# Huiweizhou/GCGCN

Measured on NVIDIA B200. Metric: document graphs/sec (fwd+bwd graph blocks), higher is better.
Workload: dtype f32

## Files before the change

### gcgcn_b200/csrc/gcn_block.cu

```cuda
#include "common.cuh"
#include "mma_tf32.cuh"

namespace gcgcn {

constexpr int BK_THREADS = 256;
constexpr int BK_WARPS = BK_THREADS / WARP;

enum { BK_OUT_DA = 0, BK_OUT_DS = 1, BK_OUT_DQ = 2 };

__device__ __forceinline__ void cp_async16(float* smem_dst, const float* gsrc) {
    const uint32_t d = static_cast<uint32_t>(__cvta_generic_to_shared(smem_dst));
    asm volatile("cp.async.cg.shared.global [%0], [%1], 16;" ::"r"(d), "l"(gsrc) : "memory");
}
__device__ __forceinline__ void cp_async_commit() { asm volatile("cp.async.commit_group;" ::: "memory"); }
template <int N>
__device__ __forceinline__ void cp_async_wait() {
    asm volatile("cp.async.wait_group %0;" ::"n"(N) : "memory");
}

__device__ __forceinline__ uint32_t s_addr(const void* p) { return static_cast<uint32_t>(__cvta_generic_to_shared(p)); }
__device__ __forceinline__ void ldsm4(uint32_t (&r)[4], const float* p) {
    asm volatile("ldmatrix.sync.aligned.m8n8.x4.shared.b16 {%0,%1,%2,%3}, [%4];"
                 : "=r"(r[0]), "=r"(r[1]), "=r"(r[2]), "=r"(r[3])
                 : "r"(s_addr(p))
// ... 194 lines not shown
        for (int r = 0; r < 8; ++r) {
            const int j = L.l8 + 8 * r;
            v[r] = -INFINITY;
            if (r < NT8 && rv && j < n) {
                v[r] = DH > 0 ? Alo[i * LDA + j] : A[abase + static_cast<long long>(i) * n + j];
                m = fmaxf(m, v[r]);
            }
        }
        float inv = 1.f;
        if (DH > 0) {
            m = group8_max(m);
            float z = 0.f;
#pragma unroll
            for (int r = 0; r < 8; ++r) {
                v[r] = (v[r] == -INFINITY) ? 0.f : __expf(v[r] - m);
                z += v[r];
            }
            z = group8_sum(z);
            inv = rv ? 1.0f / z : 0.f;
        }
        float sum = 0.f;
#pragma unroll
        for (int r = 0; r < 8; ++r) {
            const int j = L.l8 + 8 * r;
            if (r < NT8) {
                float p = 0.f;
                if (rv && j < n) {
                    p = v[r] * inv;
                    const long long pidx = abase + static_cast<long long>(i) * n + j;
                    if (DH > 0) P[pidx] = p;
                    if (drop.thr_att != 0u) p *= drop_keep(drop.seed, drop.s_att, pidx, drop.thr_att, drop.inv_att);
                }
                float hi, lo;
                split_f(p, hi, lo);
                Ahi[i * LDA + j] = hi;
                Alo[i * LDA + j] = lo;
                sum += p;
            }
        }
        sum = group8_sum(sum);
        if (L.l8 == 0) rs[i] = 1.0f / (sum + (sum == 0.f ? 1.f : 0.f));
    }

#pragma unroll
    for (int l = 0; l < layers; ++l) {
        float* Zs = Zs0 + (l & 1) * NP * LDZ;
        const int kin = l * GD;
        cp_async_wait<1>();
        __syncthreads();
        const int mt = L.warp / NG, ng = L.warp - mt * NG;
        const bool busy = L.warp < UNITS;
        const int col0 = 8 * NTW * ng;
        float c[NTW][4];
        float* zc = Zs + (16 * mt + L.g) * LDZ + col0 + 2 * L.t;
        if (l > 0) {
            if (busy) {
                const float* wb = Wf + (static_cast<size_t>(h) * layers + l) * (KI * GD * 2) + (col0 / 8) * 128 + L.lane;
#pragma unroll
                for (int nt = 0; nt < NTW; ++nt) {
                    const float2 lo2 = *reinterpret_cast<const float2*>(zc + 8 * nt);
                    const float2 hi2 = *reinterpret_cast<const float2*>(zc + 8 * LDZ + 8 * nt);
                    c[nt][0] = lo2.x; c[nt][1] = lo2.y; c[nt][2] = hi2.x; c[nt][3] = hi2.y;
                }
                const float* pa = Ghi + (16 * mt + L.a_row) * LDG + L.a_col;
#pragma unroll 2
                for (int k0 = 0; k0 < kin; k0 += 8) {
                    uint32_t ah[4], al[4];
                    ldsm4(ah, pa + k0);
                    ldsm4(al, pa + NP * LDG + k0);
#pragma unroll
                    for (int nt = 0; nt < NTW; ++nt) {
                        const float* f = wb + (k0 / 8) * (GD / 8) * 128 + nt * 128;
                        mma3(c[nt], ah, al, __float_as_uint(__ldg(f)), __float_as_uint(__ldg(f + 32)),
                             __float_as_uint(__ldg(f + 64)), __float_as_uint(__ldg(f + 96)));
                    }
                }
#pragma unroll
                for (int nt = 0; nt < NTW; ++nt) {
                    *reinterpret_cast<float2*>(zc + 8 * nt) = make_float2(c[nt][0], c[nt][1]);
                    *reinterpret_cast<float2*>(zc + 8 * LDZ + 8 * nt) = make_float2(c[nt][2], c[nt][3]);
                }
            }
            __syncthreads();
            for (int idx = tid; idx < n * CG; idx += BK_THREADS) {
                const int i = idx / CG, c4 = (idx - i * CG) * 4;
                *reinterpret_cast<float4*>(Z + hbase + (i * HD + kin + c4)) =
                    *reinterpret_cast<const float4*>(Zs + i * LDZ + c4);
            }
        }
        if (busy) {
            float2 e2[2][NTW], x2[2][NTW];
#pragma unroll
            for (int half = 0; half < 2; ++half) {
                const int i = 16 * mt + L.g + 8 * half;
#pragma unroll
                for (int nt = 0; nt < NTW; ++nt) {
                    e2[half][nt] = make_float2(0.f, 0.f);
                    x2[half][nt] = make_float2(0.f, 0.f);
                    if (i < n) {
                        const int col = col0 + 8 * nt + 2 * L.t;
                        e2[half][nt] = ld2g(Eb + (i * HD + kin + col));
                        x2[half][nt] = ld2g(xb + (i * S + kin + col));
                    }
                }
            }
#pragma unroll
            for (int nt = 0; nt < NTW; ++nt) { c[nt][0] = 0.f; c[nt][1] = 0.f; c[nt][2] = 0.f; c[nt][3] = 0.f; }
            const float* pa = Ahi + (16 * mt + L.a_row) * LDA + L.a_col;
            const float* zb = Zs + L.t * LDZ + col0 + L.g;
#pragma unroll
            for (int k0 = 0; k0 < NP; k0 += 8) {
                uint32_t ah[4], al[4];
                ldsm4(ah, pa + k0);
                ldsm4(al, pa + NP * LDA + k0);
#pragma unroll
                for (int nt = 0; nt < NTW; ++nt) mma3f(c[nt], ah, al, zb[k0 * LDZ + 8 * nt], zb[(k0 + 4) * LDZ + 8 * nt]);
            }
#pragma unroll
            for (int half = 0; half < 2; ++half) {
                const int i = 16 * mt + L.g + 8 * half;
                if (i >= n) continue;
                const float rinv = rs[i];
#pragma unroll
                for (int nt = 0; nt < NTW; ++nt) {
                    const int col = col0 + 8 * nt + 2 * L.t;
                    const int off = i * HD + kin + col;
                    float2 o;
                    o.x = fmaxf((e2[half][nt].x + c[nt][2 * half]) * rinv, 0.f);
                    o.y = fmaxf((e2[half][nt].y + c[nt][2 * half + 1]) * rinv, 0.f);
                    *reinterpret_cast<float2*>(Gb + off) = o;
                    float2 f = o;
                    if (drop.thr_gcn != 0u) {
                        const float2 k2 = drop_keep2(drop.seed, drop.s_gcn, hbase + off, drop.thr_gcn, drop.inv_gcn);
                        f.x *= k2.x; f.y *= k2.y;
                    }
                    *reinterpret_cast<float2*>(Fb + off) = make_float2(f.x + x2[half][nt].x, f.y + x2[half][nt].y);
                    if (l < layers - 1) {
                        float2 hi, lo;
                        split_f(o.x, hi.x, lo.x);
                        split_f(o.y, hi.y, lo.y);
                        *reinterpret_cast<float2*>(Ghi + i * LDG + kin + col) = hi;
                        *reinterpret_cast<float2*>(Glo + i * LDG + kin + col) = lo;
                    }
                }
            }
        }
        __syncthreads();
        if (l + 2 < layers) issue_z(l + 2);
        cp_async_commit();
    }
    cp_async_wait<0>();
}

template <int GD, int DH, int OUT, int MTC>
__global__ void __launch_bounds__(BK_THREADS, MTC <= 2 ? 4 : 3)
block_bwd_kernel(const int* __restrict__ node_ptr, const long long* __restrict__ pair_ptr,
                 const float* __restrict__ A, const float* __restrict__ q, const float* __restrict__ Z,
                 const float* __restrict__ G, const float* __restrict__ Wb, const float* __restrict__ dF,
                 float* __restrict__ dZ, float* __restrict__ dE, float* __restrict__ dOut, int heads,
                 long long total_pairs, const int* __restrict__ doc_order, int first, float scale, const BlockDrop drop) {
    extern __shared__ __align__(16) float smem[];
    const int b = doc_order != nullptr ? doc_order[first + blockIdx.x] : blockIdx.x;
    const int h = blockIdx.y;
    const int node0 = node_ptr[b];
    const int n = node_ptr[b + 1] - node0;
    if (n == 0) return;
    constexpr int S = D, layers = D / GD, CG = GD / 4, RPP = BK_THREADS / CG;
    constexpr bool SWZ = (GD == 64);
    constexpr int LDN = SWZ ? GD : GD + 12;
    constexpr int DHH = DH > 0 ? DH : 8;
    constexpr int NTW = col_tiles_per_warp(MTC, GD / 8), NG = (GD / 8) / NTW, UNITS = MTC * NG;
    constexpr int NTW_C = MTC, NG_C = 2, UNITS_C = 2 * MTC;
    constexpr int NP = 16 * MTC, MT = MTC, NT8 = 2 * MTC, LDA = NP + 4, KI = (layers - 1) * GD, LDG = KI + 4;
    const int HD = DH > 0 ? (D / DHH) * S : heads * S;

    constexpr bool TWO = (layers == 2);
    float* AtS = smem;
    float* dNh = AtS + NP * LDA;
    float* dNl = dNh + NP * LDN;
    float* Th = dNl + NP * LDN;
    float* Tl = Th + NP * LDN;
    float* rs = Tl + NP * LDN;
    float* drs = rs + NP;
    float* dAs = TWO ? Tl + NP * LDN - NP * LDA : drs + NP;
    float* dGs = TWO ? dNh : dAs + NP * LDA;
    constexpr int LDP = TWO ? LDN : LDG;

    const int tid = threadIdx.x;
    const LaneGeo L;
    auto pl = [](int row, int col) -> int {
        if (!SWZ) return row * LDN + col;
        const int mask = ((row & 3) << 1) | ((row >> 2) & 1);
        return row * LDN + ((((col >> 2) ^ mask) << 2) | (col & 3));
    };
    const long long abase = static_cast<long long>(h) * total_pairs + pair_ptr[b];
    const float* Ab = A + abase;
    const size_t hbase = static_cast<size_t>(node0) * HD + h * S;

#pragma unroll
    for (int r0 = 0; r0 < NP; r0 += 32) {
        const int i = r0 + L.rsub;
        if (i >= NP) continue;
        float sum = 0.f;
#pragma unroll
        for (int r = 0; r < 8; ++r) {
            const int j = L.l8 + 8 * r;
            if (r < NT8) {
                float v = (i < n && j < n) ? Ab[i * n + j] : 0.f;
                if (drop.thr_att != 0u && i < n && j < n)
                    v *= drop_keep(drop.seed, drop.s_att, abase + i * n + j, drop.thr_att, drop.inv_att);
                AtS[j * LDA + i] = v;
                sum += v;
            }
        }
        sum = group8_sum(sum);
        if (L.l8 == 0) { rs[i] = 1.0f / (sum + (sum == 0.f ? 1.f : 0.f)); drs[i] = 0.f; }
    }
    __syncthreads();

    const int cg = tid % CG, rg = tid / CG, c0 = cg * 4;
    float cA[NTW_C][4];
#pragma unroll
    for (int nt = 0; nt < NTW_C; ++nt) { cA[nt][0] = 0.f; cA[nt][1] = 0.f; cA[nt][2] = 0.f; cA[nt][3] = 0.f; }
#pragma unroll
    for (int l = layers - 1; l >= 0; --l) {
        const float* wsrc = Wb + (static_cast<size_t>(h) * layers + l) * (KI * GD * 2);
        const bool first_layer = (l == layers - 1);
#pragma unroll
        for (int i0 = 0; i0 < NP; i0 += RPP) {
            const int i = i0 + rg;
            if (NP % RPP != 0 && i >= NP) continue;
            float4 dn = make_float4(0.f, 0.f, 0.f, 0.f), zl = dn;
            float drp = 0.f;
            if (i < n) {
                const size_t off = hbase + (i * HD + l * GD + c0);
                float4 dg = ld4g(dF + off);
                const float4 g4 = ld4g(G + off);
                zl = ld4g(Z + off);
                if (drop.thr_gcn != 0u) {
                    const float2 k01 = drop_keep2(drop.seed, drop.s_gcn, off, drop.thr_gcn, drop.inv_gcn);
                    const float2 k23 = drop_keep2(drop.seed, drop.s_gcn, off + 2, drop.thr_gcn, drop.inv_gcn);
                    dg.x *= k01.x; dg.y *= k01.y; dg.z *= k23.x; dg.w *= k23.y;
                }
                if (!first_layer) {
                    const float4 s4 = *reinterpret_cast<const float4*>(dGs + (TWO ? pl(i, l * GD + c0) : i * LDP + l * GD + c0));
                    dg.x += s4.x; dg.y += s4.y; dg.z += s4.z; dg.w += s4.w;
                }
                dg.x = g4.x > 0.f ? dg.x : 0.f; dg.y = g4.y > 0.f ? dg.y : 0.f;
                dg.z = g4.z > 0.f ? dg.z : 0.f; dg.w = g4.w > 0.f ? dg.w : 0.f;
                const float rinv = rs[i];
                dn.x = dg.x * rinv; dn.y = dg.y * rinv; dn.z = dg.z * rinv; dn.w = dg.w * rinv;
                *reinterpret_cast<float4*>(dE + off) = dn;
                drp = -(dn.x * g4.x + dn.y * g4.y + dn.z * g4.z + dn.w * g4.w);
            }
            float4 hi, lo;
            split_f4(dn, hi, lo);
            *reinterpret_cast<float4*>(dNh + pl(i, c0)) = hi;
            *reinterpret_cast<float4*>(dNl + pl(i, c0)) = lo;
            split_f4(zl, hi, lo);
            *reinterpret_cast<float4*>(Th + pl(i, c0)) = hi;
            *reinterpret_cast<float4*>(Tl + pl(i, c0)) = lo;
#pragma unroll
            for (int o = CG / 2; o > 0; o >>= 1) drp += __shfl_xor_sync(0xffffffffu, drp, o);
            if (cg == 0 && i < n) drs[i] += drp;
        }
        __syncthreads();
        if (L.warp < UNITS_C) {
            const int mt = L.warp / NG_C, jg = L.warp - mt * NG_C;
            float (&c)[NTW_C][4] = cA;
            const int arow = 16 * mt + L.a_row, brow = 8 * NTW_C * jg + L.b_row;
            const float* pb = L.b_lo ? Tl : Th;
#pragma unroll
            for (int k0 = 0; k0 < GD; k0 += 8) {
                uint32_t ah[4], al[4];
                const float* pa = dNh + pl(arow, L.a_col + k0);
                ldsm4(ah, pa);
                ldsm4(al, pa + NP * LDN);
                const int boff = pl(brow, L.b_col + k0);
#pragma unroll
                for (int nt = 0; nt < NTW_C; ++nt) {
                    uint32_t bb[4];
                    ldsm4(bb, pb + boff + 8 * nt * LDN);
                    mma3(c[nt], ah, al, bb[0], bb[1], bb[2], bb[3]);
                }
            }
        }
        const int jt = L.warp / NG, ng = L.warp - jt * NG;
        const bool busy = L.warp < UNITS;
        const int col0 = 8 * NTW * ng;
        {
            float c[NTW][4];
#pragma unroll
            for (int nt = 0; nt < NTW; ++nt) { c[nt][0] = 0.f; c[nt][1] = 0.f; c[nt][2] = 0.f; c[nt][3] = 0.f; }
            if (busy) {
                const float* pa = AtS + (16 * jt + L.a_row) * LDA + L.a_col;
#pragma unroll
                for (int k0 = 0; k0 < NP; k0 += 8) {
                    uint32_t ah[4], al[4];
                    ldsm4(ah, pa + k0);
#pragma unroll
                    for (int e = 0; e < 4; ++e) {
                        float hi, lo;
                        split_f(__uint_as_float(ah[e]), hi, lo);
                        ah[e] = __float_as_uint(hi);
                        al[e] = __float_as_uint(lo);
                    }
#pragma unroll
                    for (int nt = 0; nt < NTW; ++nt) {
                        const float* n0 = dNh + pl(k0 + L.t, col0 + 8 * nt + L.g);
                        const float* n1 = dNh + pl(k0 + 4 + L.t, col0 + 8 * nt + L.g);
                        mma3(c[nt], ah, al, __float_as_uint(n0[0]), __float_as_uint(n1[0]), __float_as_uint(n0[NP * LDN]),
                             __float_as_uint(n1[NP * LDN]));
                    }
                }
            }
            __syncthreads();
            if (busy) {
#pragma unroll
                for (int nt = 0; nt < NTW; ++nt)
#pragma unroll
                    for (int half = 0; half < 2; ++half) {
                        const int j = 16 * jt + L.g + 8 * half, col = col0 + 8 * nt + 2 * L.t;
                        const float2 v = make_float2(c[nt][2 * half], c[nt][2 * half + 1]);
                        float2 hi, lo;
                        split_f(v.x, hi.x, lo.x);
                        split_f(v.y, hi.y, lo.y);
                        *reinterpret_cast<float2*>(Th + pl(j, col)) = hi;
                        *reinterpret_cast<float2*>(Tl + pl(j, col)) = lo;
                        if (j < n) *reinterpret_cast<float2*>(dZ + hbase + (j * HD + l * GD + col)) = v;
                    }
            }
        }
        __syncthreads();
        if (busy) {
#pragma unroll
            for (int m = 0; m < l; ++m) {
                float c[NTW][4];
#pragma unroll
                for (int nt = 0; nt < NTW; ++nt) { c[nt][0] = 0.f; c[nt][1] = 0.f; c[nt][2] = 0.f; c[nt][3] = 0.f; }
                const float* wb = wsrc + m * (GD * GD * 2) + (col0 / 8) * 128 + L.lane;
#pragma unroll 2
                for (int k0 = 0; k0 < GD; k0 += 8) {
                    uint32_t ah[4], al[4];
                    const float* pa = Th + pl(16 * jt + L.a_row, L.a_col + k0);
                    ldsm4(ah, pa);
                    ldsm4(al, pa + NP * LDN);
#pragma unroll
                    for (int nt = 0; nt < NTW; ++nt) {
                        const float* f = wb + (k0 / 8) * (GD / 8) * 128 + nt * 128;
                        mma3(c[nt], ah, al, __float_as_uint(__ldg(f)), __float_as_uint(__ldg(f + 32)),
                             __float_as_uint(__ldg(f + 64)), __float_as_uint(__ldg(f + 96)));
                    }
                }
#pragma unroll
                for (int nt = 0; nt < NTW; ++nt)
#pragma unroll
                    for (int half = 0; half < 2; ++half) {
                        float2* p = reinterpret_cast<float2*>(dGs + (TWO ? pl(16 * jt + L.g + 8 * half, m * GD + col0 + 8 * nt + 2 * L.t)
                                                                        : (16 * jt + L.g + 8 * half) * LDP + m * GD + col0 + 8 * nt + 2 * L.t));
                        float2 v = make_float2(c[nt][2 * half], c[nt][2 * half + 1]);
                        if (!first_layer) { const float2 cur = *p; v.x += cur.x; v.y += cur.y; }
                        *p = v;
                    }
            }
        }
        __syncthreads();
    }

    if (L.warp < UNITS_C) {
        const int mt = L.warp / NG_C, jg = L.warp - mt * NG_C;
#pragma unroll
        for (int nt = 0; nt < NTW_C; ++nt)
#pragma unroll
            for (int half = 0; half < 2; ++half)
                *reinterpret_cast<float2*>(dAs + (16 * mt + L.g + 8 * half) * LDA + 8 * (NTW_C * jg + nt) + 2 * L.t) =
                    make_float2(cA[nt][2 * half], cA[nt][2 * half + 1]);
    }
    __syncthreads();
#pragma unroll
    for (int r0 = 0; r0 < NP; r0 += 32) {
        const int i = r0 + L.rsub;
        if (i >= NP) continue;
        const bool rv = i < n;
        const float dr = rv ? drs[i] : 0.f;
        float p[8], dp[8];
        float dot = 0.f;
#pragma unroll
        for (int r = 0; r < 8; ++r) {
            const int j = L.l8 + 8 * r;
            p[r] = 0.f; dp[r] = 0.f;
            if (r < NT8 && rv && j < n) {
                dp[r] = dAs[i * LDA + j] + dr;
                if (OUT != BK_OUT_DA) {
                    if (drop.thr_att != 0u) {
                        dp[r] *= drop_keep(drop.seed, drop.s_att, abase + i * n + j, drop.thr_att, drop.inv_att);
                        p[r] = Ab[i * n + j];
                    } else {
                        p[r] = AtS[j * LDA + i];
                    }
                    dot += dp[r] * p[r];
                }
            }
        }
        if (OUT != BK_OUT_DA) dot = group8_sum(dot);
#pragma unroll
        for (int r = 0; r < 8; ++r) {
            const int j = L.l8 + 8 * r;
            if (r < NT8) {
                const float ds = (OUT == BK_OUT_DA) ? dp[r] : p[r] * (dp[r] - dot);
                if (OUT == BK_OUT_DQ) dAs[i * LDA + j] = ds;
                else if (rv && j < n) dOut[abase + static_cast<long long>(i) * n + j] = ds;
            }
        }
    }
    if (OUT == BK_OUT_DQ) {
        constexpr int LQ = DHH + 8, Q4 = DHH / 4;
        float* Wh = dNh;
        float* Wl = Wh + NP * LDA;
        float* qs = Wl + NP * LDA;
        for (int idx = tid; idx < NP * Q4; idx += BK_THREADS) {
            const int j = idx / Q4, k4 = (idx - j * Q4) * 4;
            float4 v = make_float4(0.f, 0.f, 0.f, 0.f);
            if (j < n) v = ld4g(q + static_cast<size_t>(node0 + j) * D + h * DHH + k4);
            *reinterpret_cast<float4*>(qs + j * LQ + k4) = v;
        }
        __syncthreads();
#pragma unroll
        for (int r0 = 0; r0 < NP; r0 += 32) {
            const int i = r0 + L.rsub;
            if (i >= NP) continue;
#pragma unroll
            for (int r = 0; r < 8; ++r) {
                const int j = L.l8 + 8 * r;
                if (r < NT8) {
                    float hi, lo;
                    split_f(dAs[i * LDA + j] + dAs[j * LDA + i], hi, lo);
                    Wh[i * LDA + j] = hi;
                    Wl[i * LDA + j] = lo;
                }
            }
        }
        __syncthreads();
        constexpr int QT = DHH / 8;
        for (int u = L.warp; u < MT * QT; u += BK_WARPS) {
            const int mt = u / QT, nt = u - mt * QT;
            float c[4] = {0.f, 0.f, 0.f, 0.f};
            const float* pa = Wh + (16 * mt + L.a_row) * LDA + L.a_col;
            const float* qb = qs + L.t * LQ + 8 * nt + L.g;
#pragma unroll
            for (int k0 = 0; k0 < NP; k0 += 8) {
                uint32_t ah[4], al[4];
                ldsm4(ah, pa + k0);
                ldsm4(al, pa + NP * LDA + k0);
                mma3f(c, ah, al, qb[k0 * LQ], qb[(k0 + 4) * LQ]);
            }
#pragma unroll
            for (int half = 0; half < 2; ++half) {
                const int i = 16 * mt + L.g + 8 * half;
                if (i < n)
                    *reinterpret_cast<float2*>(dOut + static_cast<size_t>(node0 + i) * D + h * DHH + 8 * nt + 2 * L.t) =
                        make_float2(c[2 * half] * scale, c[2 * half + 1] * scale);
            }
        }
    }
}

static size_t block_fwd_smem(int np, int layers, int gd) {
    const int ki = (layers - 1) * gd;
    return (2 * static_cast<size_t>(np) * (np + 4) + 2 * static_cast<size_t>(np) * (gd + 8) +
            2 * static_cast<size_t>(np) * (ki + 4) + np) * sizeof(float);
}
static size_t block_bwd_smem(int np, int layers, int gd) {
    const int ki = (layers - 1) * gd;
    size_t fl = static_cast<size_t>(np) * (np + 4) + 4 * static_cast<size_t>(np) * (gd == 64 ? gd : gd + 12) + 2 * np;
    if (layers != 2) fl += static_cast<size_t>(np) * (np + 4) + static_cast<size_t>(np) * (ki + 4);
    return fl * sizeof(float);
}

bool block_kernels_usable(const gcgcn_batch* bt, int heads, int layers, int slab, bool mha) {
    if (slab != D || layers < 1 || slab % layers != 0) return false;
    const int gd = slab / layers;
    if (bt->max_nodes > 64 || !(gd == 32 || gd == 64)) return false;
    if (mha) {
        if (heads < 1 || D % heads != 0) return false;
        const int dh = D / heads;
        if (!(dh == 16 || dh == 32)) return false;
    }
    return true;
}

template <int GD, int DH, int MTC>
static int launch_fwd_class(const gcgcn_batch* bt, int heads, int count, int first, const int* order, const float* A,
                            const float* q, float* P, float* Z, const float* E, const float* Winner, const float* x,
                            float* G, float* F, float scale, const BlockDrop& drop, cudaStream_t st) {
    constexpr int layers = D / GD;
    const size_t smem = block_fwd_smem(16 * MTC, layers, GD);
    static std::atomic<unsigned long long> prepared{0};
    GCGCN_TRY(set_smem_once(prepared, block_fwd_kernel<GD, DH, MTC>, smem, "block_fwd"));
    block_fwd_kernel<GD, DH, MTC><<<dim3(count, heads), BK_THREADS, smem, st>>>(
        bt->node_ptr, reinterpret_cast<const long long*>(bt->pair_ptr), A, q, P, Z, E, Winner, x, G, F, heads,
        bt->total_pairs, order, first, scale, drop);
    GCGCN_CHECK_LAUNCH(DH > 0 ? "block_fwd<mha>" : "block_fwd<given>");
    return GCGCN_OK;
}

template <int GD, int DH>
static int launch_fwd_all(const gcgcn_batch* bt, int heads, const float* A, const float* q, float* P, float* Z,
                          const float* E, const float* Winner, const float* x, float* G, float* F, float scale,
                          const BlockDrop& drop, cudaStream_t st) {
    return for_each_size_class(bt, [&](int count, int first, int nmax, const int* order) -> int {
        switch ((nmax + 15) / 16) {
            case 1: return launch_fwd_class<GD, DH, 1>(bt, heads, count, first, order, A, q, P, Z, E, Winner, x, G, F, scale, drop, st);
            case 2: return launch_fwd_class<GD, DH, 2>(bt, heads, count, first, order, A, q, P, Z, E, Winner, x, G, F, scale, drop, st);
            case 3: return launch_fwd_class<GD, DH, 3>(bt, heads, count, first, order, A, q, P, Z, E, Winner, x, G, F, scale, drop, st);
            case 4: return launch_fwd_class<GD, DH, 4>(bt, heads, count, first, order, A, q, P, Z, E, Winner, x, G, F, scale, drop, st);
            default: return fail(GCGCN_ERR_UNSUPPORTED, "block_fwd: %d nodes > 64", nmax);
        }
    });
}

static int launch_winner_frag(const float* Winner, int heads, int layers, float* frag_ws, cudaStream_t st) {
    if (layers < 2) return GCGCN_OK;
    if (frag_ws == nullptr) return fail(GCGCN_ERR_WORKSPACE, "block kernels: no workspace for the fragment-ordered weights");
    const size_t half = block_frag_floats(heads, layers) / 2;
    winner_frag_kernel<<<dim3(heads * layers, 8), 256, 0, st>>>(Winner, layers, D / layers, frag_ws, frag_ws + half);
    GCGCN_CHECK_LAUNCH("winner_frag");
    return GCGCN_OK;
}

bool tile_blocks_enabled();
size_t tile_wblob_bytes(int heads);
int launch_tile_fwd(const gcgcn_batch* bt, int heads, int layers, const float* q, float* P, float* Z, const float* E,
                    const float* Winner_rowmajor, const float* x, float* G, float* F, void* wblob_ws, cudaStream_t st);

int launch_block_fwd(const gcgcn_batch* bt, int heads, int layers, const float* A, const float* q, float* P,
                     float* Z, const float* E, const float* Winner_rowmajor, const float* x, float* G, float* F,
                     float* frag_ws, const BlockDrop& drop, cudaStream_t st) {
    if (bt->num_docs == 0) return GCGCN_OK;
    if (A == nullptr && layers == 2 && (heads == 8 || heads == 4) && drop.thr_att == 0u && drop.thr_gcn == 0u && bt->tile_doc != nullptr &&
        bt->num_tiles > 0 && bt->row_doc != nullptr && frag_ws != nullptr &&
        tile_wblob_bytes(heads) <= block_frag_floats(heads, layers) * sizeof(float) && tile_blocks_enabled())
        return launch_tile_fwd(bt, heads, layers, q, P, Z, E, Winner_rowmajor, x, G, F, frag_ws, st);
    GCGCN_TRY(launch_winner_frag(Winner_rowmajor, heads, layers, frag_ws, st));
    const float* Winner = frag_ws;
    const int gd = D / layers;
    const int dh = A != nullptr ? 0 : D / heads;
    const float scale = dh > 0 ? 1.0f / sqrtf(static_cast<float>(dh)) : 1.f;
#define GCGCN_BK_FWD(GD_, DH_) \
    if (gd == GD_ && dh == DH_) return launch_fwd_all<GD_, DH_>(bt, heads, A, q, P, Z, E, Winner, x, G, F, scale, drop, st);
    GCGCN_BK_FWD(64, 0)
    GCGCN_BK_FWD(64, 16)
    GCGCN_BK_FWD(64, 32)
    GCGCN_BK_FWD(32, 0)
    GCGCN_BK_FWD(32, 16)
    GCGCN_BK_FWD(32, 32)
#undef GCGCN_BK_FWD
    return fail(GCGCN_ERR_UNSUPPORTED, "block_fwd: sub-layer width %d / head width %d not supported", gd, dh);
}

template <int GD, int DH, int OUT, int MTC>
static int launch_bwd_class(const gcgcn_batch* bt, int heads, int count, int first, const int* order, const float* A,
                            const float* q, const float* Z, const float* G, const float* Winner, const float* dF,
                            float* dZ, float* dE, float* dOut, float scale, const BlockDrop& drop, cudaStream_t st) {
    constexpr int layers = D / GD;
    const size_t smem = block_bwd_smem(16 * MTC, layers, GD);
    static std::atomic<unsigned long long> prepared{0};
    GCGCN_TRY(set_smem_once(prepared, block_bwd_kernel<GD, DH, OUT, MTC>, smem, "block_bwd"));
    block_bwd_kernel<GD, DH, OUT, MTC><<<dim3(count, heads), BK_THREADS, smem, st>>>(
        bt->node_ptr, reinterpret_cast<const long long*>(bt->pair_ptr), A, q, Z, G, Winner, dF, dZ, dE, dOut, heads,
        bt->total_pairs, order, first, scale, drop);
    GCGCN_CHECK_LAUNCH(OUT == BK_OUT_DQ ? "block_bwd<dq>" : (OUT == BK_OUT_DS ? "block_bwd<dS>" : "block_bwd<dA>"));
    return GCGCN_OK;
}

template <int GD, int DH, int OUT>
static int launch_bwd_all(const gcgcn_batch* bt, int heads, const float* A, const float* q, const float* Z,
                          const float* G, const float* Winner, const float* dF, float* dZ, float* dE, float* dOut,
                          float scale, const BlockDrop& drop, cudaStream_t st) {
    return for_each_size_class(bt, [&](int count, int first, int nmax, const int* order) -> int {
        switch ((nmax + 15) / 16) {
            case 1: return launch_bwd_class<GD, DH, OUT, 1>(bt, heads, count, first, order, A, q, Z, G, Winner, dF, dZ, dE, dOut, scale, drop, st);
            case 2: return launch_bwd_class<GD, DH, OUT, 2>(bt, heads, count, first, order, A, q, Z, G, Winner, dF, dZ, dE, dOut, scale, drop, st);
            case 3: return launch_bwd_class<GD, DH, OUT, 3>(bt, heads, count, first, order, A, q, Z, G, Winner, dF, dZ, dE, dOut, scale, drop, st);
            case 4: return launch_bwd_class<GD, DH, OUT, 4>(bt, heads, count, first, order, A, q, Z, G, Winner, dF, dZ, dE, dOut, scale, drop, st);
            default: return fail(GCGCN_ERR_UNSUPPORTED, "block_bwd: %d nodes > 64", nmax);
        }
    });
}

int launch_block_bwd(const gcgcn_batch* bt, int heads, int layers, int out_mode, const float* A, const float* q,
                     const float* Z, const float* G, const float* Winner_rowmajor, const float* dF, float* dZ, float* dE,
                     float* dOut, float* frag_ws, const BlockDrop& drop, cudaStream_t st) {
    if (bt->num_docs == 0) return GCGCN_OK;
    GCGCN_TRY(launch_winner_frag(Winner_rowmajor, heads, layers, frag_ws, st));
    const float* Winner = frag_ws == nullptr ? nullptr : frag_ws + block_frag_floats(heads, layers) / 2;
    const int gd = D / layers;
    const int dh = out_mode == BK_OUT_DQ ? D / heads : 0;
    const float scale = dh > 0 ? 1.0f / sqrtf(static_cast<float>(dh)) : 1.f;
#define GCGCN_BK_BWD(GD_, DH_, OUT_)                      \
    if (gd == GD_ && dh == DH_ && out_mode == OUT_)       \
        return launch_bwd_all<GD_, DH_, OUT_>(bt, heads, A, q, Z, G, Winner, dF, dZ, dE, dOut, scale, drop, st);
    GCGCN_BK_BWD(64, 0, BK_OUT_DA)
    GCGCN_BK_BWD(32, 0, BK_OUT_DA)
    GCGCN_BK_BWD(64, 0, BK_OUT_DS)
    GCGCN_BK_BWD(32, 0, BK_OUT_DS)
    GCGCN_BK_BWD(64, 16, BK_OUT_DQ)
    GCGCN_BK_BWD(64, 32, BK_OUT_DQ)
    GCGCN_BK_BWD(32, 16, BK_OUT_DQ)
    GCGCN_BK_BWD(32, 32, BK_OUT_DQ)
#undef GCGCN_BK_BWD
    return fail(GCGCN_ERR_UNSUPPORTED, "block_bwd: sub-layer width %d / head width %d / mode %d not supported", gd, dh,
                out_mode);
}

}
```

Before: 900,600.

## Make backward graph-block kernel persistent with cp.async prefetch ring and staged row stores

Converts the backward block kernel into a persistent grid sized by occupancy that loops over (document, head) items. For small graphs it prefetches the next item's attention matrix and the per-layer dF/G/Z slabs into a shared-memory ring with cp.async, overlapping loads with compute. dZ and dq outputs are staged in shared memory and written as coalesced float4 rows. Costs are extra shared memory, which can lower occupancy, and a lower launch-bounds CTA count for MTC=4.

Result: no change. 899,400 (median of 6 runs) (-0.1%).

```diff
diff --git a/gcgcn_b200/csrc/gcn_block.cu b/gcgcn_b200/csrc/gcn_block.cu
--- a/gcgcn_b200/csrc/gcn_block.cu
+++ b/gcgcn_b200/csrc/gcn_block.cu
@@ -370,19 +370,36 @@
     cp_async_wait<0>();
 }
 
+__host__ __device__ constexpr bool bwd_ring(int np) { return np <= 16; }
+#ifndef XROWS
+#define XROWS 1
+#endif
+#ifndef XPERSIST
+#define XPERSIST 1
+#endif
+__host__ __device__ constexpr int bwd_core_floats(int np, int layers, int gd) {
+    return np * (np + 4) + 4 * np * (gd == 64 ? gd : gd + 12) + 2 * np +
+           (layers == 2 ? 0 : np * (np + 4) + np * ((layers - 1) * gd + 4));
+}
+__host__ __device__ constexpr int bwd_smem_floats(int np, int layers, int gd) {
+    return bwd_core_floats(np, layers, gd) + (bwd_ring(np) ? 3 * np * gd + np * np : 0);
+}
+
+__device__ __forceinline__ void cp_async4(float* smem_dst, const float* gsrc) {
+    const uint32_t d = static_cast<uint32_t>(__cvta_generic_to_shared(smem_dst));
+    asm volatile("cp.async.ca.shared.global [%0], [%1], 4;" ::"r"(d), "l"(gsrc) : "memory");
+}
+__device__ __forceinline__ float join_f(float hi, float lo) { return lo == 0.f ? hi : hi + lo; }
+
 template <int GD, int DH, int OUT, int MTC>
-__global__ void __launch_bounds__(BK_THREADS, MTC <= 2 ? 4 : 3)
+__global__ void __launch_bounds__(BK_THREADS, MTC <= 2 ? 4 : (MTC == 3 ? 3 : 2))
 block_bwd_kernel(const int* __restrict__ node_ptr, const long long* __restrict__ pair_ptr,
                  const float* __restrict__ A, const float* __restrict__ q, const float* __restrict__ Z,
                  const float* __restrict__ G, const float* __restrict__ Wb, const float* __restrict__ dF,
                  float* __restrict__ dZ, float* __restrict__ dE, float* __restrict__ dOut, int heads,
-                 long long total_pairs, const int* __restrict__ doc_order, int first, float scale, const BlockDrop drop) {
+                 long long total_pairs, const int* __restrict__ doc_order, int first, int count, float scale,
+                 const BlockDrop drop) {
     extern __shared__ __align__(16) float smem[];
-    const int b = doc_order != nullptr ? doc_order[first + blockIdx.x] : blockIdx.x;
-    const int h = blockIdx.y;
-    const int node0 = node_ptr[b];
-    const int n = node_ptr[b + 1] - node0;
-    if (n == 0) return;
     constexpr int S = D, layers = D / GD, CG = GD / 4, RPP = BK_THREADS / CG;
     constexpr bool SWZ = (GD == 64);
     constexpr int LDN = SWZ ? GD : GD + 12;
@@ -390,6 +407,8 @@
     constexpr int NTW = col_tiles_per_warp(MTC, GD / 8), NG = (GD / 8) / NTW, UNITS = MTC * NG;
     constexpr int NTW_C = MTC, NG_C = 2, UNITS_C = 2 * MTC;
     constexpr int NP = 16 * MTC, MT = MTC, NT8 = 2 * MTC, LDA = NP + 4, KI = (layers - 1) * GD, LDG = KI + 4;
+    constexpr bool RING = bwd_ring(NP);
+    constexpr bool ROWS = XROWS;
     const int HD = DH > 0 ? (D / DHH) * S : heads * S;
 
     constexpr bool TWO = (layers == 2);
@@ -403,6 +422,8 @@
     float* dAs = TWO ? Tl + NP * LDN - NP * LDA : drs + NP;
     float* dGs = TWO ? dNh : dAs + NP * LDA;
     constexpr int LDP = TWO ? LDN : LDG;
+    float* Rs = smem + bwd_core_floats(NP, layers, GD);
+    float* Ar = Rs + 3 * NP * GD;
 
     const int tid = threadIdx.x;
     const LaneGeo L;
@@ -411,276 +432,349 @@
         const int mask = ((row & 3) << 1) | ((row >> 2) & 1);
         return row * LDN + ((((col >> 2) ^ mask) << 2) | (col & 3));
     };
-    const long long abase = static_cast<long long>(h) * total_pairs + pair_ptr[b];
-    const float* Ab = A + abase;
-    const size_t hbase = static_cast<size_t>(node0) * HD + h * S;
-
-#pragma unroll
-    for (int r0 = 0; r0 < NP; r0 += 32) {
-        const int i = r0 + L.rsub;
-        if (i >= NP) continue;
-        float sum = 0.f;
-#pragma unroll
-        for (int r = 0; r < 8; ++r) {
-            const int j = L.l8 + 8 * r;
-            if (r < NT8) {
-                float v = (i < n && j < n) ? Ab[i * n + j] : 0.f;
-                if (drop.thr_att != 0u && i < n && j < n)
-                    v *= drop_keep(drop.seed, drop.s_att, abase + i * n + j, drop.thr_att, drop.inv_att);
-                AtS[j * LDA + i] = v;
-                sum += v;
-            }
-        }
-        sum = group8_sum(sum);
-        if (L.l8 == 0) { rs[i] = 1.0f / (sum + (sum == 0.f ? 1.f : 0.f)); drs[i] = 0.f; }
-    }
-    __syncthreads();
+    struct Item {
+        int node0, n, h;
+        long long abase;
+        size_t hbase;
+    };
+    auto item_at = [&](int it) -> Item {
+        Item w;
+        const int d = it % count;
+        w.h = it / count;
+        const int b = doc_order != nullptr ? doc_order[first + d] : d;
+        w.node0 = node_ptr[b];
+        w.n = node_ptr[b + 1] - w.node0;
+        w.abase = static_cast<long long>(w.h) * total_pairs + pair_ptr[b];
+        w.hbase = static_cast<size_t>(w.node0) * HD + w.h * S;
+        return w;
+    };
+    auto issue_layer = [&](const Item& w, int l) {
+        if (RING)
+        for (int idx = tid; idx < w.n * CG; idx += BK_THREADS) {
+            const int i = idx / CG, c4 = (idx - i * CG) * 4;
+            const size_t off = w.hbase + (i * HD + l * GD + c4);
+            cp_async16(Rs + i * GD + c4, dF + off);
+            cp_async16(Rs + NP * GD + i * GD + c4, G + off);
+            cp_async16(Rs + 2 * NP * GD + i * GD + c4, Z + off);
+        }
+    };
+    const int items = count * heads;
+    auto issue_item = [&](int it) {
+        if (RING && it < items) {
+            const Item w = item_at(it);
+            const float* src = A + w.abase;
+            for (int k = tid; k < w.n * w.n; k += BK_THREADS) cp_async4(Ar + k, src + k);
+            issue_layer(w, layers - 1);
+        }
+        cp_async_commit();
+    };
+    issue_item(blockIdx.x);
 
     const int cg = tid % CG, rg = tid / CG, c0 = cg * 4;
-    float cA[NTW_C][4];
-#pragma unroll
-    for (int nt = 0; nt < NTW_C; ++nt) { cA[nt][0] = 0.f; cA[nt][1] = 0.f; cA[nt][2] = 0.f; cA[nt][3] = 0.f; }
-#pragma unroll
-    for (int l = layers - 1; l >= 0; --l) {
-        const float* wsrc = Wb + (static_cast<size_t>(h) * layers + l) * (KI * GD * 2);
-        const bool first_layer = (l == layers - 1);
-#pragma unroll
-        for (int i0 = 0; i0 < NP; i0 += RPP) {
-            const int i = i0 + rg;
-            if (NP % RPP != 0 && i >= NP) continue;
-            float4 dn = make_float4(0.f, 0.f, 0.f, 0.f), zl = dn;
-            float drp = 0.f;
-            if (i < n) {
-                const size_t off = hbase + (i * HD + l * GD + c0);
-                float4 dg = ld4g(dF + off);
-                const float4 g4 = ld4g(G + off);
-                zl = ld4g(Z + off);
-                if (drop.thr_gcn != 0u) {
-                    const float2 k01 = drop_keep2(drop.seed, drop.s_gcn, off, drop.thr_gcn, drop.inv_gcn);
-                    const float2 k23 = drop_keep2(drop.seed, drop.s_gcn, off + 2, drop.thr_gcn, drop.inv_gcn);
-                    dg.x *= k01.x; dg.y *= k01.y; dg.z *= k23.x; dg.w *= k23.y;
-                }
-                if (!first_layer) {
-                    const float4 s4 = *reinterpret_cast<const float4*>(dGs + (TWO ? pl(i, l * GD + c0) : i * LDP + l * GD + c0));
-                    dg.x += s4.x; dg.y += s4.y; dg.z += s4.z; dg.w += s4.w;
-                }
-                dg.x = g4.x > 0.f ? dg.x : 0.f; dg.y = g4.y > 0.f ? dg.y : 0.f;
-                dg.z = g4.z > 0.f ? dg.z : 0.f; dg.w = g4.w > 0.f ? dg.w : 0.f;
-                const float rinv = rs[i];
-                dn.x = dg.x * rinv; dn.y = dg.y * rinv; dn.z = dg.z * rinv; dn.w = dg.w * rinv;
-                *reinterpret_cast<float4*>(dE + off) = dn;
-                drp = -(dn.x * g4.x + dn.y * g4.y + dn.z * g4.z + dn.w * g4.w);
-            }
-            float4 hi, lo;
-            split_f4(dn, hi, lo);
-            *reinterpret_cast<float4*>(dNh + pl(i, c0)) = hi;
-            *reinterpret_cast<float4*>(dNl + pl(i, c0)) = lo;
-            split_f4(zl, hi, lo);
-            *reinterpret_cast<float4*>(Th + pl(i, c0)) = hi;
-            *reinterpret_cast<float4*>(Tl + pl(i, c0)) = lo;
-#pragma unroll
-            for (int o = CG / 2; o > 0; o >>= 1) drp += __shfl_xor_sync(0xffffffffu, drp, o);
-            if (cg == 0 && i < n) drs[i] += drp;
-        }
+    for (int it = blockIdx.x; it < items; it += gridDim.x) {
+        const Item w = item_at(it);
+        const int n = w.n, h = w.h, node0 = w.node0;
+        const long long abase = w.abase;
+        const float* Ab = A + abase;
+        const size_t hbase = w.hbase;
+        cp_async_wait<0>();
         __syncthreads();
+        if (n == 0) {
+            issue_item(it + gridDim.x);
+            continue;
+        }
+
+#pragma unroll
+        for (int r0 = 0; r0 < NP; r0 += 32) {
+            const int i = r0 + L.rsub;
+            if (i >= NP) continue;
+            float sum = 0.f;
+#pragma unroll
+            for (int r = 0; r < 8; ++r) {
+                const int j = L.l8 + 8 * r;
+                if (r < NT8) {
+                    float v = (i < n && j < n) ? (RING ? Ar[i * n + j] : Ab[i * n + j]) : 0.f;
+                    if (drop.thr_att != 0u && i < n && j < n)
+                        v *= drop_keep(drop.seed, drop.s_att, abase + i * n + j, drop.thr_att, drop.inv_att);
+                    AtS[j * LDA + i] = v;
+                    sum += v;
+                }
+            }
+            sum = group8_sum(sum);
+            if (L.l8 == 0) { rs[i] = 1.0f / (sum + (sum == 0.f ? 1.f : 0.f)); drs[i] = 0.f; }
+        }
+        __syncthreads();
+
+        float cA[NTW_C][4];
+#pragma unroll
+        for (int nt = 0; nt < NTW_C; ++nt) { cA[nt][0] = 0.f; cA[nt][1] = 0.f; cA[nt][2] = 0.f; cA[nt][3] = 0.f; }
+#pragma unroll
+        for (int l = layers - 1; l >= 0; --l) {
+            const float* wsrc = Wb + (static_cast<size_t>(h) * layers + l) * (KI * GD * 2);
+            const bool first_layer = (l == layers - 1);
+#pragma unroll
+            for (int i0 = 0; i0 < NP; i0 += RPP) {
+                const int i = i0 + rg;
+                if (NP % RPP != 0 && i >= NP) continue;
+                float4 dn = make_float4(0.f, 0.f, 0.f, 0.f), zl = dn;
+                float drp = 0.f;
+                if (i < n) {
+                    const size_t off = hbase + (i * HD + l * GD + c0);
+                    const float* rrow = Rs + i * GD + c0;
+                    float4 dg = RING ? *reinterpret_cast<const float4*>(rrow) : ld4g(dF + off);
+                    const float4 g4 = RING ? *reinterpret_cast<const float4*>(rrow + NP * GD) : ld4g(G + off);
+                    zl = RING ? *reinterpret_cast<const float4*>(rrow + 2 * NP * GD) : ld4g(Z + off);
+                    if (drop.thr_gcn != 0u) {
+                        const float2 k01 = drop_keep2(drop.seed, drop.s_gcn, off, drop.thr_gcn, drop.inv_gcn);
+                        const float2 k23 = drop_keep2(drop.seed, drop.s_gcn, off + 2, drop.thr_gcn, drop.inv_gcn);
+                        dg.x *= k01.x; dg.y *= k01.y; dg.z *= k23.x; dg.w *= k23.y;
+                    }
+                    if (!first_layer) {
+                        const float4 s4 = *reinterpret_cast<const float4*>(dGs + (TWO ? pl(i, l * GD + c0) : i * LDP + l * GD + c0));
+                        dg.x += s4.x; dg.y += s4.y; dg.z += s4.z; dg.w += s4.w;
+                    }
+                    dg.x = g4.x > 0.f ? dg.x : 0.f; dg.y = g4.y > 0.f ? dg.y : 0.f;
+                    dg.z = g4.z > 0.f ? dg.z : 0.f; dg.w = g4.w > 0.f ? dg.w : 0.f;
+                    const float rinv = rs[i];
+                    dn.x = dg.x * rinv; dn.y = dg.y * rinv; dn.z = dg.z * rinv; dn.w = dg.w * rinv;
+                    *reinterpret_cast<float4*>(dE + off) = dn;
+                    drp = -(dn.x * g4.x + dn.y * g4.y + dn.z * g4.z + dn.w * g4.w);
+                }
+                float4 hi, lo;
+                split_f4(dn, hi, lo);
+                *reinterpret_cast<float4*>(dNh + pl(i, c0)) = hi;
+                *reinterpret_cast<float4*>(dNl + pl(i, c0)) = lo;
+                split_f4(zl, hi, lo);
+                *reinterpret_cast<float4*>(Th + pl(i, c0)) = hi;
+                *reinterpret_cast<float4*>(Tl + pl(i, c0)) = lo;
+#pragma unroll
+                for (int o = CG / 2; o > 0; o >>= 1) drp += __shfl_xor_sync(0xffffffffu, drp, o);
+                if (cg == 0 && i < n) drs[i] += drp;
+            }
+            __syncthreads();
+            if (l > 0) {
+                issue_layer(w, l - 1);
+                cp_async_commit();
+            } else {
+                issue_item(it + gridDim.x);
+            }
+            if (L.warp < UNITS_C) {
+                const int mt = L.warp / NG_C, jg = L.warp - mt * NG_C;
+                float (&c)[NTW_C][4] = cA;
+                const int arow = 16 * mt + L.a_row, brow = 8 * NTW_C * jg + L.b_row;
+                const float* pb = L.b_lo ? Tl : Th;
+#pragma unroll
+                for (int k0 = 0; k0 < GD; k0 += 8) {
+                    uint32_t ah[4], al[4];
+                    const float* pa = dNh + pl(arow, L.a_col + k0);
+                    ldsm4(ah, pa);
+                    ldsm4(al, pa + NP * LDN);
+                    const int boff = pl(brow, L.b_col + k0);
+#pragma unroll
+                    for (int nt = 0; nt < NTW_C; ++nt) {
+                        uint32_t bb[4];
+                        ldsm4(bb, pb + boff + 8 * nt * LDN);
+                        mma3(c[nt], ah, al, bb[0], bb[1], bb[2], bb[3]);
+                    }
+                }
+            }
+            const int jt = L.warp / NG, ng = L.warp - jt * NG;
+            const bool busy = L.warp < UNITS;
+            const int col0 = 8 * NTW * ng;
+            {
+                float c[NTW][4];
+#pragma unroll
+                for (int nt = 0; nt < NTW; ++nt) { c[nt][0] = 0.f; c[nt][1] = 0.f; c[nt][2] = 0.f; c[nt][3] = 0.f; }
+                if (busy) {
+                    const float* pa = AtS + (16 * jt + L.a_row) * LDA + L.a_col;
+#pragma unroll
+                    for (int k0 = 0; k0 < NP; k0 += 8) {
+                        uint32_t ah[4], al[4];
+                        ldsm4(ah, pa + k0);
+#pragma unroll
+                        for (int e = 0; e < 4; ++e) {
+                            float hi, lo;
+                            split_f(__uint_as_float(ah[e]), hi, lo);
+                            ah[e] = __float_as_uint(hi);
+                            al[e] = __float_as_uint(lo);
+                        }
+#pragma unroll
+                        for (int nt = 0; nt < NTW; ++nt) {
+                            const float* n0 = dNh + pl(k0 + L.t, col0 + 8 * nt + L.g);
+                            const float* n1 = dNh + pl(k0 + 4 + L.t, col0 + 8 * nt + L.g);
+                            mma3(c[nt], ah, al, __float_as_uint(n0[0]), __float_as_uint(n1[0]), __float_as_uint(n0[NP * LDN]),
+                                 __float_as_uint(n1[NP * LDN]));
+                        }
+                    }
+                }
+                __syncthreads();
+                if (busy) {
+#pragma unroll
+                    for (int nt = 0; nt < NTW; ++nt)
+#pragma unroll
+                        for (int half = 0; half < 2; ++half) {
+                            const int j = 16 * jt + L.g + 8 * half, col = col0 + 8 * nt + 2 * L.t;
+                            float2 hi, lo;
+                            split_f(c[nt][2 * half], hi.x, lo.x);
+                            split_f(c[nt][2 * half + 1], hi.y, lo.y);
+                            *reinterpret_cast<float2*>(Th + pl(j, col)) = hi;
+                            *reinterpret_cast<float2*>(Tl + pl(j, col)) = lo;
+                            if (!ROWS && j < n) *reinterpret_cast<float2*>(dZ + hbase + (j * HD + l * GD + col)) = make_float2(c[nt][2 * half], c[nt][2 * half + 1]);
+                        }
+                }
+            }
+            __syncthreads();
+            if (ROWS)
+            for (int idx = tid; idx < n * CG; idx += BK_THREADS) {
+                const int j = idx / CG, c4 = (idx - j * CG) * 4;
+                const float4 hi = *reinterpret_cast<const float4*>(Th + pl(j, c4));
+                const float4 lo = *reinterpret_cast<const float4*>(Tl + pl(j, c4));
+                *reinterpret_cast<float4*>(dZ + hbase + (j * HD + l * GD + c4)) =
+                    make_float4(join_f(hi.x, lo.x), join_f(hi.y, lo.y), join_f(hi.z, lo.z), join_f(hi.w, lo.w));
+            }
+            if (busy) {
+#pragma unroll
+                for (int m = 0; m < l; ++m) {
+                    float c[NTW][4];
+#pragma unroll
+                    for (int nt = 0; nt < NTW; ++nt) { c[nt][0] = 0.f; c[nt][1] = 0.f; c[nt][2] = 0.f; c[nt][3] = 0.f; }
+                    const float* wb = wsrc + m * (GD * GD * 2) + (col0 / 8) * 128 + L.lane;
+#pragma unroll 2
+                    for (int k0 = 0; k0 < GD; k0 += 8) {
+                        uint32_t ah[4], al[4];
+                        const float* pa = Th + pl(16 * jt + L.a_row, L.a_col + k0);
+                        ldsm4(ah, pa);
+                        ldsm4(al, pa + NP * LDN);
+#pragma unroll
+                        for (int nt = 0; nt < NTW; ++nt) {
+                            const float* f = wb + (k0 / 8) * (GD / 8) * 128 + nt * 128;
+                            mma3(c[nt], ah, al, __float_as_uint(__ldg(f)), __float_as_uint(__ldg(f + 32)),
+                                 __float_as_uint(__ldg(f + 64)), __float_as_uint(__ldg(f + 96)));
+                        }
+                    }
+#pragma unroll
+                    for (int nt = 0; nt < NTW; ++nt)
+#pragma unroll
+                        for (int half = 0; half < 2; ++half) {
+                            float2* p = reinterpret_cast<float2*>(dGs + (TWO ? pl(16 * jt + L.g + 8 * half, m * GD + col0 + 8 * nt + 2 * L.t)
+                                                                            : (16 * jt + L.g + 8 * half) * LDP + m * GD + col0 + 8 * nt + 2 * L.t));
+                            float2 v = make_float2(c[nt][2 * half], c[nt][2 * half + 1]);
+                            if (!first_layer) { const float2 cur = *p; v.x += cur.x; v.y += cur.y; }
+                            *p = v;
+                        }
+                }
+            }
+            if (l > 0) cp_async_wait<0>();
+            __syncthreads();
+        }
+
         if (L.warp < UNITS_C) {
             const int mt = L.warp / NG_C, jg = L.warp - mt * NG_C;
-            float (&c)[NTW_C][4] = cA;
-            const int arow = 16 * mt + L.a_row, brow = 8 * NTW_C * jg + L.b_row;
-            const float* pb = L.b_lo ? Tl : Th;
-#pragma unroll
-            for (int k0 = 0; k0 < GD; k0 += 8) {
-                uint32_t ah[4], al[4];
-                const float* pa = dNh + pl(arow, L.a_col + k0);
-                ldsm4(ah, pa);
-                ldsm4(al, pa + NP * LDN);
-                const int boff = pl(brow, L.b_col + k0);
-#pragma unroll
-                for (int nt = 0; nt < NTW_C; ++nt) {
-                    uint32_t bb[4];
-                    ldsm4(bb, pb + boff + 8 * nt * LDN);
-                    mma3(c[nt], ah, al, bb[0], bb[1], bb[2], bb[3]);
-                }
-            }
-        }
-        const int jt = L.warp / NG, ng = L.warp - jt * NG;
-        const bool busy = L.warp < UNITS;
-        const int col0 = 8 * NTW * ng;
-        {
-            float c[NTW][4];
-#pragma unroll
-            for (int nt = 0; nt < NTW; ++nt) { c[nt][0] = 0.f; c[nt][1] = 0.f; c[nt][2] = 0.f; c[nt][3] = 0.f; }
-            if (busy) {
-                const float* pa = AtS + (16 * jt + L.a_row) * LDA + L.a_col;
+#pragma unroll
+            for (int nt = 0; nt < NTW_C; ++nt)
+#pragma unroll
+                for (int half = 0; half < 2; ++half)
+                    *reinterpret_cast<float2*>(dAs + (16 * mt + L.g + 8 * half) * LDA + 8 * (NTW_C * jg + nt) + 2 * L.t) =
+                        make_float2(cA[nt][2 * half], cA[nt][2 * half + 1]);
+        }
+        __syncthreads();
+#pragma unroll
+        for (int r0 = 0; r0 < NP; r0 += 32) {
+            const int i = r0 + L.rsub;
+            if (i >= NP) continue;
+            const bool rv = i < n;
+            const float dr = rv ? drs[i] : 0.f;
+            float p[8], dp[8];
+            float dot = 0.f;
+#pragma unroll
+            for (int r = 0; r < 8; ++r) {
+                const int j = L.l8 + 8 * r;
+                p[r] = 0.f; dp[r] = 0.f;
+                if (r < NT8 && rv && j < n) {
+                    dp[r] = dAs[i * LDA + j] + dr;
+                    if (OUT != BK_OUT_DA) {
+                        if (drop.thr_att != 0u) {
+                            dp[r] *= drop_keep(drop.seed, drop.s_att, abase + i * n + j, drop.thr_att, drop.inv_att);
+                            p[r] = Ab[i * n + j];
+                        } else {
+                            p[r] = AtS[j * LDA + i];
+                        }
+                        dot += dp[r] * p[r];
+                    }
+                }
+            }
+            if (OUT != BK_OUT_DA) dot = group8_sum(dot);
+#pragma unroll
+            for (int r = 0; r < 8; ++r) {
+                const int j = L.l8 + 8 * r;
+                if (r < NT8) {
+                    const float ds = (OUT == BK_OUT_DA) ? dp[r] : p[r] * (dp[r] - dot);
+                    if (OUT == BK_OUT_DQ) dAs[i * LDA + j] = ds;
+                    else if (rv && j < n) dOut[abase + static_cast<long long>(i) * n + j] = ds;
+                }
+            }
+        }
+        if (OUT == BK_OUT_DQ) {
+            constexpr int LQ = DHH + 8, Q4 = DHH / 4;
+            float* Wh = dNh;
+            float* Wl = Wh + NP * LDA;
+            float* qs = Wl + NP * LDA;
+            float* dqs = qs + NP * LQ;
+            static_assert(NP * LDA + NP * (2 * LDA + 2 * LQ) <= bwd_core_floats(NP, layers, GD), "dq scratch");
+            for (int idx = tid; idx < NP * Q4; idx += BK_THREADS) {
+                const int j = idx / Q4, k4 = (idx - j * Q4) * 4;
+                float4 v = make_float4(0.f, 0.f, 0.f, 0.f);
+                if (j < n) v = ld4g(q + static_cast<size_t>(node0 + j) * D + h * DHH + k4);
+                *reinterpret_cast<float4*>(qs + j * LQ + k4) = v;
+            }
+            __syncthreads();
+#pragma unroll
+            for (int r0 = 0; r0 < NP; r0 += 32) {
+                const int i = r0 + L.rsub;
+                if (i >= NP) continue;
+#pragma unroll
+                for (int r = 0; r < 8; ++r) {
+                    const int j = L.l8 + 8 * r;
+                    if (r < NT8) {
+                        float hi, lo;
+                        split_f(dAs[i * LDA + j] + dAs[j * LDA + i], hi, lo);
+                        Wh[i * LDA + j] = hi;
+                        Wl[i * LDA + j] = lo;
+                    }
+                }
+            }
+            __syncthreads();
+            constexpr int QT = DHH / 8;
+            for (int u = L.warp; u < MT * QT; u += BK_WARPS) {
+                const int mt = u / QT, nt = u - mt * QT;
+                float c[4] = {0.f, 0.f, 0.f, 0.f};
+                const float* pa = Wh + (16 * mt + L.a_row) * LDA + L.a_col;
+                const float* qb = qs + L.t * LQ + 8 * nt + L.g;
 #pragma unroll
                 for (int k0 = 0; k0 < NP; k0 += 8) {
                     uint32_t ah[4], al[4];
                     ldsm4(ah, pa + k0);
-#pragma unroll
-                    for (int e = 0; e < 4; ++e) {
-                        float hi, lo;
-                        split_f(__uint_as_float(ah[e]), hi, lo);
-                        ah[e] = __float_as_uint(hi);
-                        al[e] = __float_as_uint(lo);
-                    }
-#pragma unroll
-                    for (int nt = 0; nt < NTW; ++nt) {
-                        const float* n0 = dNh + pl(k0 + L.t, col0 + 8 * nt + L.g);
-                        const float* n1 = dNh + pl(k0 + 4 + L.t, col0 + 8 * nt + L.g);
-                        mma3(c[nt], ah, al, __float_as_uint(n0[0]), __float_as_uint(n1[0]), __float_as_uint(n0[NP * LDN]),
-                             __float_as_uint(n1[NP * LDN]));
-                    }
-                }
-            }
-            __syncthreads();
-            if (busy) {
-#pragma unroll
-                for (int nt = 0; nt < NTW; ++nt)
-#pragma unroll
-                    for (int half = 0; half < 2; ++half) {
-                        const int j = 16 * jt + L.g + 8 * half, col = col0 + 8 * nt + 2 * L.t;
-                        const float2 v = make_float2(c[nt][2 * half], c[nt][2 * half + 1]);
-                        float2 hi, lo;
-                        split_f(v.x, hi.x, lo.x);
-                        split_f(v.y, hi.y, lo.y);
-                        *reinterpret_cast<float2*>(Th + pl(j, col)) = hi;
-                        *reinterpret_cast<float2*>(Tl + pl(j, col)) = lo;
-                        if (j < n) *reinterpret_cast<float2*>(dZ + hbase + (j * HD + l * GD + col)) = v;
-                    }
-            }
-        }
-        __syncthreads();
-        if (busy) {
-#pragma unroll
-            for (int m = 0; m < l; ++m) {
-                float c[NTW][4];
-#pragma unroll
-                for (int nt = 0; nt < NTW; ++nt) { c[nt][0] = 0.f; c[nt][1] = 0.f; c[nt][2] = 0.f; c[nt][3] = 0.f; }
-                const float* wb = wsrc + m * (GD * GD * 2) + (col0 / 8) * 128 + L.lane;
-#pragma unroll 2
-                for (int k0 = 0; k0 < GD; k0 += 8) {
-                    uint32_t ah[4], al[4];
-                    const float* pa = Th + pl(16 * jt + L.a_row, L.a_col + k0);
-                    ldsm4(ah, pa);
-                    ldsm4(al, pa + NP * LDN);
-#pragma unroll
-                    for (int nt = 0; nt < NTW; ++nt) {
-                        const float* f = wb + (k0 / 8) * (GD / 8) * 128 + nt * 128;
-                        mma3(c[nt], ah, al, __float_as_uint(__ldg(f)), __float_as_uint(__ldg(f + 32)),
-                             __float_as_uint(__ldg(f + 64)), __float_as_uint(__ldg(f + 96)));
-                    }
-                }
-#pragma unroll
-                for (int nt = 0; nt < NTW; ++nt)
-#pragma unroll
-                    for (int half = 0; half < 2; ++half) {
-                        float2* p = reinterpret_cast<float2*>(dGs + (TWO ? pl(16 * jt + L.g + 8 * half, m * GD + col0 + 8 * nt + 2 * L.t)
-                                                                        : (16 * jt + L.g + 8 * half) * LDP + m * GD + col0 + 8 * nt + 2 * L.t));
-                        float2 v = make_float2(c[nt][2 * half], c[nt][2 * half + 1]);
-                        if (!first_layer) { const float2 cur = *p; v.x += cur.x; v.y += cur.y; }
-                        *p = v;
-                    }
-            }
-        }
-        __syncthreads();
+                    ldsm4(al, pa + NP * LDA + k0);
+                    mma3f(c, ah, al, qb[k0 * LQ], qb[(k0 + 4) * LQ]);
+                }
+#pragma unroll
+                for (int half = 0; half < 2; ++half) {
+                    if (ROWS) *reinterpret_cast<float2*>(dqs + (16 * mt + L.g + 8 * half) * LQ + 8 * nt + 2 * L.t) =
+                        make_float2(c[2 * half] * scale, c[2 * half + 1] * scale);
+                    else if (16 * mt + L.g + 8 * half < n)
+                    *reinterpret_cast<float2*>(dOut + static_cast<size_t>(node0 + 16 * mt + L.g + 8 * half) * D + h * DHH + 8 * nt + 2 * L.t) =
+                        make_float2(c[2 * half] * scale, c[2 * half + 1] * scale);
+                }
+            }
+            if (ROWS) __syncthreads();
+            if (ROWS) for (int idx = tid; idx < n * Q4; idx += BK_THREADS) {
+                const int i = idx / Q4, k4 = (idx - i * Q4) * 4;
+                *reinterpret_cast<float4*>(dOut + static_cast<size_t>(node0 + i) * D + h * DHH + k4) =
+                    *reinterpret_cast<const float4*>(dqs + i * LQ + k4);
+            }
+        }
     }
-
-    if (L.warp < UNITS_C) {
-        const int mt = L.warp / NG_C, jg = L.warp - mt * NG_C;
-#pragma unroll
-        for (int nt = 0; nt < NTW_C; ++nt)
-#pragma unroll
-            for (int half = 0; half < 2; ++half)
-                *reinterpret_cast<float2*>(dAs + (16 * mt + L.g + 8 * half) * LDA + 8 * (NTW_C * jg + nt) + 2 * L.t) =
-                    make_float2(cA[nt][2 * half], cA[nt][2 * half + 1]);
-    }
-    __syncthreads();
-#pragma unroll
-    for (int r0 = 0; r0 < NP; r0 += 32) {
-        const int i = r0 + L.rsub;
-        if (i >= NP) continue;
-        const bool rv = i < n;
-        const float dr = rv ? drs[i] : 0.f;
-        float p[8], dp[8];
-        float dot = 0.f;
-#pragma unroll
-        for (int r = 0; r < 8; ++r) {
-            const int j = L.l8 + 8 * r;
-            p[r] = 0.f; dp[r] = 0.f;
-            if (r < NT8 && rv && j < n) {
-                dp[r] = dAs[i * LDA + j] + dr;
-                if (OUT != BK_OUT_DA) {
-                    if (drop.thr_att != 0u) {
-                        dp[r] *= drop_keep(drop.seed, drop.s_att, abase + i * n + j, drop.thr_att, drop.inv_att);
-                        p[r] = Ab[i * n + j];
-                    } else {
-                        p[r] = AtS[j * LDA + i];
-                    }
-                    dot += dp[r] * p[r];
-                }
-            }
-        }
-        if (OUT != BK_OUT_DA) dot = group8_sum(dot);
-#pragma unroll
-        for (int r = 0; r < 8; ++r) {
-            const int j = L.l8 + 8 * r;
-            if (r < NT8) {
-                const float ds = (OUT == BK_OUT_DA) ? dp[r] : p[r] * (dp[r] - dot);
-                if (OUT == BK_OUT_DQ) dAs[i * LDA + j] = ds;
-                else if (rv && j < n) dOut[abase + static_cast<long long>(i) * n + j] = ds;
-            }
-        }
-    }
-    if (OUT == BK_OUT_DQ) {
-        constexpr int LQ = DHH + 8, Q4 = DHH / 4;
-        float* Wh = dNh;
-        float* Wl = Wh + NP * LDA;
-        float* qs = Wl + NP * LDA;
-        for (int idx = tid; idx < NP * Q4; idx += BK_THREADS) {
-            const int j = idx / Q4, k4 = (idx - j * Q4) * 4;
-            float4 v = make_float4(0.f, 0.f, 0.f, 0.f);
-            if (j < n) v = ld4g(q + static_cast<size_t>(node0 + j) * D + h * DHH + k4);
-            *reinterpret_cast<float4*>(qs + j * LQ + k4) = v;
-        }
-        __syncthreads();
-#pragma unroll
-        for (int r0 = 0; r0 < NP; r0 += 32) {
-            const int i = r0 + L.rsub;
-            if (i >= NP) continue;
-#pragma unroll
-            for (int r = 0; r < 8; ++r) {
-                const int j = L.l8 + 8 * r;
-                if (r < NT8) {
-                    float hi, lo;
-                    split_f(dAs[i * LDA + j] + dAs[j * LDA + i], hi, lo);
-                    Wh[i * LDA + j] = hi;
-                    Wl[i * LDA + j] = lo;
-                }
-            }
-        }
-        __syncthreads();
-        constexpr int QT = DHH / 8;
-        for (int u = L.warp; u < MT * QT; u += BK_WARPS) {
-            const int mt = u / QT, nt = u - mt * QT;
-            float c[4] = {0.f, 0.f, 0.f, 0.f};
-            const float* pa = Wh + (16 * mt + L.a_row) * LDA + L.a_col;
-            const float* qb = qs + L.t * LQ + 8 * nt + L.g;
-#pragma unroll
-            for (int k0 = 0; k0 < NP; k0 += 8) {
-                uint32_t ah[4], al[4];
-                ldsm4(ah, pa + k0);
-                ldsm4(al, pa + NP * LDA + k0);
-                mma3f(c, ah, al, qb[k0 * LQ], qb[(k0 + 4) * LQ]);
-            }
-#pragma unroll
-            for (int half = 0; half < 2; ++half) {
-                const int i = 16 * mt + L.g + 8 * half;
-                if (i < n)
-                    *reinterpret_cast<float2*>(dOut + static_cast<size_t>(node0 + i) * D + h * DHH + 8 * nt + 2 * L.t) =
-                        make_float2(c[2 * half] * scale, c[2 * half + 1] * scale);
-            }
-        }
-    }
+    cp_async_wait<0>();
 }
 
 static size_t block_fwd_smem(int np, int layers, int gd) {
@@ -689,10 +783,7 @@
             2 * static_cast<size_t>(np) * (ki + 4) + np) * sizeof(float);
 }
 static size_t block_bwd_smem(int np, int layers, int gd) {
-    const int ki = (layers - 1) * gd;
-    size_t fl = static_cast<size_t>(np) * (np + 4) + 4 * static_cast<size_t>(np) * (gd == 64 ? gd : gd + 12) + 2 * np;
-    if (layers != 2) fl += static_cast<size_t>(np) * (np + 4) + static_cast<size_t>(np) * (ki + 4);
-    return fl * sizeof(float);
+    return static_cast<size_t>(bwd_smem_floats(np, layers, gd)) * sizeof(float);
 }
 
 bool block_kernels_usable(const gcgcn_batch* bt, int heads, int layers, int slab, bool mha) {
@@ -781,12 +872,24 @@
                             const float* q, const float* Z, const float* G, const float* Winner, const float* dF,
                             float* dZ, float* dE, float* dOut, float scale, const BlockDrop& drop, cudaStream_t st) {
     constexpr int layers = D / GD;
+    const auto kernel = block_bwd_kernel<GD, DH, OUT, MTC>;
     const size_t smem = block_bwd_smem(16 * MTC, layers, GD);
-    static std::atomic<unsigned long long> prepared{0};
-    GCGCN_TRY(set_smem_once(prepared, block_bwd_kernel<GD, DH, OUT, MTC>, smem, "block_bwd"));
-    block_bwd_kernel<GD, DH, OUT, MTC><<<dim3(count, heads), BK_THREADS, smem, st>>>(
+    static std::atomic<int> resident[64];
+    int dev = 0;
+    GCGCN_TRY(cuda_ok(cudaGetDevice(&dev), "block_bwd"));
+    if (dev < 0 || dev >= 64) return fail(GCGCN_ERR_CUDA, "block_bwd: device ordinal %d out of range", dev);
+    int ctas = resident[dev].load(std::memory_order_acquire);
+    if (ctas == 0) {
+        GCGCN_TRY(set_smem(kernel, smem, "block_bwd"));
+        int per_sm = 0;
+        GCGCN_TRY(cuda_ok(cudaOccupancyMaxActiveBlocksPerMultiprocessor(&per_sm, kernel, BK_THREADS, smem), "block_bwd"));
+        ctas = std::max(per_sm, 1) * sm_count();
+        resident[dev].store(ctas, std::memory_order_release);
+    }
+    const long long items = static_cast<long long>(count) * heads;
+    kernel<<<static_cast<int>((XPERSIST || MTC == 1) ? std::min<long long>(items, ctas) : items), BK_THREADS, smem, st>>>(
         bt->node_ptr, reinterpret_cast<const long long*>(bt->pair_ptr), A, q, Z, G, Winner, dF, dZ, dE, dOut, heads,
-        bt->total_pairs, order, first, scale, drop);
+        bt->total_pairs, order, first, count, scale, drop);
     GCGCN_CHECK_LAUNCH(OUT == BK_OUT_DQ ? "block_bwd<dq>" : (OUT == BK_OUT_DS ? "block_bwd<dS>" : "block_bwd<dA>"));
     return GCGCN_OK;
 }
```
